# ubc-vision/quadraturefields

Hardware: AMD Instinct MI355X
Metric: rays/sec at 800x800 Lego (mesh-quadrature render: ray/mesh intersection + hash-grid/MLP field + compositing) (higher is better)
Workload: dtype f32; 1 GPU; Lego 800x800 (configs[1]), 1xMI355X per frame, fp32 hash-grid + tiny-MLP HIP kernels; rays_per_frame=640000, max_hits=25, triangles=983040, log2_hashmap_size=19, up_sample=1, bvh_fallback_frames=0, overflow_repaired_frames=8, reorigin_rule_redone_frames=0, camera_mismatch_frames=0, frames_in_flight=1

## Files before the change

### quadraturefields_amd/csrc/raster.hip

```cpp
#include <type_traits>

#include "exact_common.h"

#pragma clang fp contract(off)

namespace {

struct RasterCam {
    float r00, r01, r02, r10, r11, r12, r20, r21, r22;
    float cx, cy, cz;
    float fx, fy, px0, py0;
    int w, h;
};

constexpr float kRasterGuard = 0.25f;

struct SlabArgs {
    float t_lo, t_hi;
    int stop_at;
    uint64_t *keys;
    const float4 *ray_rec;
};

struct TriSetup {
    int x0, x1, y0, y1;
    bool use_edges;
    float ea[3], eb[3], ec[3];
};

__device__ __forceinline__ bool tri_setup(const float4 a, const float4 b, const float4 c, const RasterCam &cam, TriSetup &s)
{
    float minx = INFINITY, maxx = -INFINITY, miny = INFINITY, maxy = -INFINITY;
    int behind = 0;
    const float4 vs[3] = {a, b, c};
    float sxs[3], sys[3];
#pragma unroll
    for (int k = 0; k < 3; ++k) {
        const float dx = vs[k].x - cam.cx, dy = vs[k].y - cam.cy, dz = vs[k].z - cam.cz;
        const float xc = cam.r00 * dx + cam.r10 * dy + cam.r20 * dz;
        const float yc = cam.r01 * dx + cam.r11 * dy + cam.r21 * dz;
        const float zc = cam.r02 * dx + cam.r12 * dy + cam.r22 * dz;
        const float zv = -zc;
        if (!(zv > 1e-6f)) { ++behind; sxs[k] = sys[k] = 0.0f; continue; }
        const float sx = cam.fx * (xc / zv) + cam.px0;
        const float sy = -cam.fy * (yc / zv) + cam.py0;
        sxs[k] = sx; sys[k] = sy;
        minx = fminf(minx, sx); maxx = fmaxf(maxx, sx);
        miny = fminf(miny, sy); maxy = fmaxf(maxy, sy);
    }
    if (behind == 3) return false;
    s.use_edges = false;
    if (behind > 0) {
        s.x0 = 0; s.y0 = 0; s.x1 = cam.w - 1; s.y1 = cam.h - 1;
    } else {
        s.x0 = (int)fmaxf(floorf(minx - kRasterGuard), 0.0f);
        s.y0 = (int)fmaxf(floorf(miny - kRasterGuard), 0.0f);
        s.x1 = (int)fminf(ceilf(maxx + kRasterGuard), (float)(cam.w - 1));
        s.y1 = (int)fminf(ceilf(maxy + kRasterGuard), (float)(cam.h - 1));
        if (!(maxx + kRasterGuard >= 0.0f) || !(maxy + kRasterGuard >= 0.0f) ||
            !(minx - kRasterGuard <= (float)(cam.w - 1)) || !(miny - kRasterGuard <= (float)(cam.h - 1)))
            return false;
        const float area2 = (sxs[1] - sxs[0]) * (sys[2] - sys[0]) - (sys[1] - sys[0]) * (sxs[2] - sxs[0]);
        if (fabsf(area2) > 1e-2f) {
            s.use_edges = true;
            const float sgn = area2 > 0.0f ? 1.0f : -1.0f;
#pragma unroll
            for (int k = 0; k < 3; ++k) {
                const int k1 = (k + 1) % 3;
                const float ex = sxs[k1] - sxs[k], ey = sys[k1] - sys[k];
                s.ea[k] = -sgn * ey;
                s.eb[k] = sgn * ex;
                s.ec[k] = -(s.ea[k] * sxs[k] + s.eb[k] * sys[k]) + (kRasterGuard + 0.05f) * (fabsf(ex) + fabsf(ey)) + 1e-3f;
            }
        }
    }
    return true;
}

constexpr int kBinStage = 256;
constexpr int kBinIdBits = 26;
struct BinStage { int n; int tile[kBinStage]; uint2 rec[kBinStage]; };
struct TileBins {
    int32_t *cursor;
    uint2 *bins;
    int cap;
    BinStage *stage;
};

__device__ __forceinline__ void bin_records(const TileBins &tb, int tile, uint2 rec)
{
    const int lane = (int)__lane_id();
    for (;;) {
        const int t0 = __builtin_amdgcn_readfirstlane(tile);
        const unsigned long long m = __ballot(tile == t0);
        if (tile == t0) {
            const int rank = __popcll(m & ((1ull << lane) - 1ull));
            int base = 0;
            if (rank == 0) base = atomicAdd(&tb.cursor[t0], __popcll(m));
            base = __shfl(base, __ffsll((long long)m) - 1, 64);
            if (base + rank < tb.cap) tb.bins[(int64_t)t0 * tb.cap + base + rank] = rec;
            break;
        }
    }
}

template <int kRasterLanes, bool kWide, bool kSlab = false, bool kBins = false>
__device__ __forceinline__ void raster_triangle(const float4 *__restrict__ tris, int64_t tri_i, int sub, const RasterCam &cam,
                                                const float *__restrict__ rays_o, const float *__restrict__ rays_d,
                                                int max_hits, int32_t *__restrict__ hit_tri, float *__restrict__ hit_t,
                                                int32_t *__restrict__ hit_count, int32_t *__restrict__ overflow,
                                                const bool cam_origin, const SlabArgs slab = SlabArgs(),
                                                const TileBins bins = TileBins())
{
    const float4 a = tris[tri_i * 3 + 0], b = tris[tri_i * 3 + 1], c = tris[tri_i * 3 + 2];
    const int id = __float_as_int(a.w);
    TriSetup ts;
    if (!tri_setup(a, b, c, cam, ts)) return;
    const int x0 = ts.x0, x1 = ts.x1, y0 = ts.y0, y1 = ts.y1;
    const bool use_edges = ts.use_edges;
    const float *ea = ts.ea, *eb = ts.eb, *ec = ts.ec;
    const int bw = x1 - x0 + 1;
    const int total = bw * (y1 - y0 + 1);
    int px = x0 + sub % bw, py = y0 + sub / bw;
    for (int q = sub; q < total; q += kRasterLanes) {
        const int cx_ = px, cy_ = py;
        px += kRasterLanes;
        while (px > x1) { px -= bw; ++py; }
        if (use_edges) {
            const float fx_ = (float)cx_, fy_ = (float)cy_;
            if (ea[0] * fx_ + eb[0] * fy_ + ec[0] < 0.0f || ea[1] * fx_ + eb[1] * fy_ + ec[1] < 0.0f ||
                ea[2] * fx_ + eb[2] * fy_ + ec[2] < 0.0f)
                continue;
        }
        const int64_t ray = (int64_t)cy_ * cam.w + cx_;
        float dx, dy, dz;
        if (kSlab && slab.ray_rec) {
            const float4 rr = slab.ray_rec[ray];
            if (__float_as_int(rr.w) >= slab.stop_at) continue;
            dx = rr.x; dy = rr.y; dz = rr.z;
        } else {
            dx = rays_d[ray * 3]; dy = rays_d[ray * 3 + 1]; dz = rays_d[ray * 3 + 2];
        }
        float ox = cam.cx, oy = cam.cy, oz = cam.cz;
        if (!cam_origin) { ox = rays_o[ray * 3]; oy = rays_o[ray * 3 + 1]; oz = rays_o[ray * 3 + 2]; }
        asm volatile("" : "+v"(ox), "+v"(oy), "+v"(oz), "+v"(dx), "+v"(dy), "+v"(dz));
        float t;
        if (!mt_hit(a, b, c, ox, oy, oz, dx, dy, dz, &t)) continue;
        if (kSlab) {
            if (!(t >= slab.t_lo && t < slab.t_hi)) continue;
            const int slot = atomicAdd(&hit_count[ray], 1);
            if (slot < max_hits) slab.keys[(int64_t)slot * ((int64_t)cam.w * cam.h) + ray] = hit_key(t, id);
            else atomicAdd(overflow, 1);
            continue;
        }
        if (kBins) {
            const int tile = (cy_ >> 3) * ((cam.w + 7) >> 3) + (cx_ >> 3);
            const uint2 rec = make_uint2(__float_as_uint(t), ((uint32_t)id << 6) | (uint32_t)((cy_ & 7) * 8 + (cx_ & 7)));
            const int at = atomicAdd(&bins.stage->n, 1);
            if (at < kBinStage) { bins.stage->tile[at] = tile; bins.stage->rec[at] = rec; }
            else bin_records(bins, tile, rec);
            continue;
        }
        const int slot = atomicAdd(&hit_count[ray], 1);
        if (slot < max_hits) {
            const int64_t at = kWide ? (int64_t)slot * ((int64_t)cam.w * cam.h) + ray : ray * max_hits + slot;
            hit_t[at] = t;
            if (hit_tri) hit_tri[at] = id;
        } else {
            atomicAdd(overflow, 1);
        }
    }
}

template <int kRasterLanes, bool kWide>
__global__ __launch_bounds__(256) void raster_kernel(const float4 *__restrict__ tris, int64_t n_tri, RasterCam cam,
                                                     const float *__restrict__ rays_o, const float *__restrict__ rays_d,
                                                     int max_hits, int32_t *__restrict__ hit_tri, float *__restrict__ hit_t,
                                                     int32_t *__restrict__ hit_count, int32_t *__restrict__ overflow,
                                                     const int32_t *__restrict__ ray_flag)
{
    const int64_t gid = (int64_t)blockIdx.x * blockDim.x + threadIdx.x;
    const int64_t tri_i = gid / kRasterLanes;
    const int sub = (int)(gid % kRasterLanes);
    if (tri_i >= n_tri) return;
    if (ray_flag && *ray_flag) return;
    const bool cam_origin = ray_flag != nullptr;
    raster_triangle<kRasterLanes, kWide>(tris, tri_i, sub, cam, rays_o, rays_d, max_hits, hit_tri, hit_t, hit_count, overflow,
                                         cam_origin);
}

template <int kRasterLanes>
__global__ __launch_bounds__(256) void raster_bins_kernel(const float4 *__restrict__ tris, int64_t n_tri, RasterCam cam,
                                                          const float *__restrict__ rays_o, const float *__restrict__ rays_d,
                                                          int max_hits, int32_t *__restrict__ tile_cursor,
                                                          uint2 *__restrict__ bin_records_out,
                                                          const int32_t *__restrict__ ray_flag)
{
    __shared__ BinStage s_stage[4];
    const int64_t gid = (int64_t)blockIdx.x * blockDim.x + threadIdx.x;
    const int64_t tri_i = gid / kRasterLanes;
    const int sub = (int)(gid % kRasterLanes);
    if (ray_flag && *ray_flag) return;
    const bool cam_origin = ray_flag != nullptr;
    const int lane = (int)(threadIdx.x & 63);
    TileBins tb;
    tb.cursor = tile_cursor;
    tb.bins = bin_records_out;
    tb.cap = 64 * max_hits;
    tb.stage = &s_stage[threadIdx.x >> 6];
    if (lane == 0) tb.stage->n = 0;
    __builtin_amdgcn_fence(__ATOMIC_ACQ_REL, "workgroup");
    __builtin_amdgcn_wave_barrier();
    if (tri_i < n_tri)
        raster_triangle<kRasterLanes, false, false, true>(tris, tri_i, sub, cam, rays_o, rays_d, max_hits, nullptr, nullptr,
                                                          nullptr, nullptr, cam_origin, SlabArgs(), tb);
    __builtin_amdgcn_fence(__ATOMIC_ACQ_REL, "workgroup");
    __builtin_amdgcn_wave_barrier();
    const int n = tb.stage->n < kBinStage ? tb.stage->n : kBinStage;
    for (int i = lane; i < n; i += 64) bin_records(tb, tb.stage->tile[i], tb.stage->rec[i]);
}

__global__ __launch_bounds__(64) void tile_count_kernel(const int32_t *__restrict__ tile_cursor, const uint2 *__restrict__ bins,
                                                        int max_hits, int w, int h, int tiles_x,
                                                        int32_t *__restrict__ hit_count, int32_t *__restrict__ overflow,
                                                        uint64_t *__restrict__ tile_mask)
{
    __shared__ int s_cnt[64];
    const int tile = blockIdx.x, lane = threadIdx.x;
    const int cap = 64 * max_hits;
    const int cursor = tile_cursor[tile];
    const int n = cursor < cap ? cursor : cap;
    const int px = (tile % tiles_x) * 8 + (lane & 7), py = (tile / tiles_x) * 8 + (lane >> 3);
    const bool inside = px < w && py < h;
    int c = 0;
    if (n > 0) {
        s_cnt[lane] = 0;
        __syncthreads();
        const uint2 *run = bins + (int64_t)tile * cap;
        for (int i = lane; i < n; i += 64) atomicAdd(&s_cnt[run[i].y & 63u], 1);
        __syncthreads();
        c = s_cnt[lane];
    }
    int over = c > max_hits ? c - max_hits : 0;
    if (cursor > cap) {
        c = c > max_hits ? c : max_hits + 1;
        over = lane == 0 ? cursor - cap : 0;
    }
    if (inside) hit_count[(int64_t)py * w + px] = c;
    const unsigned long long mask = __ballot(inside && c > max_hits);
    if (mask) {
#pragma unroll
        for (int off = 32; off > 0; off >>= 1) over += __shfl_xor(over, off, 64);
        if (lane == 0) atomicAdd(overflow, over);
    }
    if (lane == 0) tile_mask[tile] = mask;
}

constexpr float kRayPixelTol = 0.02f;
constexpr float kRayUnitTol = 1e-4f;

__device__ __forceinline__ void camera_rays_check(const uint32_t *__restrict__ o_bits, const float *__restrict__ rays_d,
                                                  int64_t n_rays, const RasterCam &cam, int32_t *__restrict__ flag,
                                                  int64_t first, int64_t stride)
{
    const uint32_t c0 = __float_as_uint(cam.cx), c1 = __float_as_uint(cam.cy), c2 = __float_as_uint(cam.cz);
    bool bad = false;
    for (int64_t r = first; r < n_rays; r += stride) {
        const uint32_t o0 = o_bits[r * 3], o1 = o_bits[r * 3 + 1], o2 = o_bits[r * 3 + 2];
        const float dx = rays_d[r * 3], dy = rays_d[r * 3 + 1], dz = rays_d[r * 3 + 2];
        bad = bad || o0 != c0 || o1 != c1 || o2 != c2;
        const float xc = cam.r00 * dx + cam.r10 * dy + cam.r20 * dz;
        const float yc = cam.r01 * dx + cam.r11 * dy + cam.r21 * dz;
        const float zv = -(cam.r02 * dx + cam.r12 * dy + cam.r22 * dz);
        const float sx = cam.fx * (xc / zv) + cam.px0, sy = -cam.fy * (yc / zv) + cam.py0;
        const float px = (float)(int)(r % cam.w), py = (float)(int)(r / cam.w);
        bad = bad || !(zv > 0.0f) || !(fabsf(sx - px) <= kRayPixelTol) || !(fabsf(sy - py) <= kRayPixelTol) ||
              !(fabsf(dx * dx + dy * dy + dz * dz - 1.0f) <= kRayUnitTol);
    }
    if (bad) *flag = 1;
}

__global__ void camera_rays_check_kernel(const uint32_t *__restrict__ o_bits, const float *__restrict__ rays_d, int64_t n_rays,
                                         RasterCam cam, int32_t *__restrict__ flag)
{
    camera_rays_check(o_bits, rays_d, n_rays, cam, flag, (int64_t)blockIdx.x * blockDim.x + threadIdx.x,
                      (int64_t)gridDim.x * blockDim.x);
}

constexpr int kCullChunk = 64;

__global__ __launch_bounds__(256) void chunk_boxes_kernel(const float4 *__restrict__ tris, int64_t n_tri, int n_chunks,
                                                          float4 *__restrict__ boxes)
{
    const int chunk = (int)(((int64_t)blockIdx.x * blockDim.x + threadIdx.x) >> 6), lane = threadIdx.x & 63;
    if (chunk >= n_chunks) return;
    const int64_t t = (int64_t)chunk * kCullChunk + lane;
    float lo[3] = {INFINITY, INFINITY, INFINITY}, hi[3] = {-INFINITY, -INFINITY, -INFINITY};
    if (t < n_tri) {
#pragma unroll
        for (int k = 0; k < 3; ++k) {
            const float4 v = tris[t * 3 + k];
            lo[0] = fminf(lo[0], v.x); lo[1] = fminf(lo[1], v.y); lo[2] = fminf(lo[2], v.z);
            hi[0] = fmaxf(hi[0], v.x); hi[1] = fmaxf(hi[1], v.y); hi[2] = fmaxf(hi[2], v.z);
        }
    }
#pragma unroll
    for (int off = 32; off > 0; off >>= 1) {
#pragma unroll
        for (int k = 0; k < 3; ++k) {
            lo[k] = fminf(lo[k], __shfl_xor(lo[k], off, 64));
            hi[k] = fmaxf(hi[k], __shfl_xor(hi[k], off, 64));
        }
    }
    if (lane == 0) {
        boxes[chunk * 2 + 0] = make_float4(lo[0], lo[1], lo[2], 0.0f);
        boxes[chunk * 2 + 1] = make_float4(hi[0], hi[1], hi[2], 0.0f);
    }
}

__global__ void cull_chunks_kernel(const float4 *__restrict__ boxes, int n_chunks, RasterCam cam, int32_t *__restrict__ visible,
                                   int32_t *__restrict__ counters, int parity, const uint32_t *__restrict__ o_bits,
                                   const float *__restrict__ rays_d, int64_t n_rays, int32_t *__restrict__ ray_flag)
{
    const int chunk = blockIdx.x * blockDim.x + threadIdx.x;
    if (chunk == 0) counters[parity ^ 1] = 0;
    if (ray_flag) camera_rays_check(o_bits, rays_d, n_rays, cam, ray_flag, chunk, (int64_t)gridDim.x * blockDim.x);
    if (chunk >= n_chunks) return;
    const float4 lo = boxes[chunk * 2], hi = boxes[chunk * 2 + 1];
    if (!(lo.x <= hi.x)) return;
    float minx = INFINITY, maxx = -INFINITY, miny = INFINITY, maxy = -INFINITY;
    bool keep = false;
#pragma unroll
    for (int k = 0; k < 8; ++k) {
        const float dx = ((k & 1) ? hi.x : lo.x) - cam.cx, dy = ((k & 2) ? hi.y : lo.y) - cam.cy, dz = ((k & 4) ? hi.z : lo.z) - cam.cz;
        const float xc = cam.r00 * dx + cam.r10 * dy + cam.r20 * dz;
        const float yc = cam.r01 * dx + cam.r11 * dy + cam.r21 * dz;
        const float zc = cam.r02 * dx + cam.r12 * dy + cam.r22 * dz;
        const float zv = -zc;
        if (!(zv > 1e-4f)) { keep = true; continue; }
        const float sx = cam.fx * (xc / zv) + cam.px0, sy = -cam.fy * (yc / zv) + cam.py0;
        minx = fminf(minx, sx); maxx = fmaxf(maxx, sx);
        miny = fminf(miny, sy); maxy = fmaxf(maxy, sy);
    }
    const float g = kRasterGuard + 1.0f;
    if (!keep)
        keep = (maxx + g >= 0.0f) && (maxy + g >= 0.0f) && (minx - g <= (float)(cam.w - 1)) && (miny - g <= (float)(cam.h - 1));
    if (keep) visible[atomicAdd(&counters[parity], 1)] = chunk;
}

template <int kRasterLanes, bool kWide>
__global__ __launch_bounds__(256) void raster_culled_kernel(const float4 *__restrict__ tris, int64_t n_tri, RasterCam cam,
                                                            const float *__restrict__ rays_o, const float *__restrict__ rays_d,
                                                            int max_hits, int32_t *__restrict__ hit_tri, float *__restrict__ hit_t,
                                                            int32_t *__restrict__ hit_count, int32_t *__restrict__ overflow,
                                                            const int32_t *__restrict__ visible, const int32_t *__restrict__ n_visible,
                                                            const int32_t *__restrict__ ray_flag)
{
    if (ray_flag && *ray_flag) return;
    const bool cam_origin = ray_flag != nullptr;
    constexpr int kTrisPerBlock = 256 / kRasterLanes;
    constexpr int kBlocksPerChunk = kCullChunk / kTrisPerBlock;
    const int n_items = *n_visible * kBlocksPerChunk;
    const int sub = threadIdx.x % kRasterLanes;
    for (int item = blockIdx.x; item < n_items; item += gridDim.x) {
        const int chunk = visible[item / kBlocksPerChunk];
        const int64_t tri_i = (int64_t)chunk * kCullChunk + (item % kBlocksPerChunk) * kTrisPerBlock + threadIdx.x / kRasterLanes;
        if (tri_i < n_tri)
            raster_triangle<kRasterLanes, kWide>(tris, tri_i, sub, cam, rays_o, rays_d, max_hits, hit_tri, hit_t, hit_count, overflow,
                                                 cam_origin);
    }
}

// ... 372 lines not shown
        bvh->chunk_dirty = true;
        bvh->cull_parity = 0;
    }
    if (bvh->chunk_dirty) {
        hipLaunchKernelGGL(chunk_boxes_kernel, dim3((unsigned)qf_div_up(n_chunks * 64, 256)), dim3(256), 0, st,
                           reinterpret_cast<const float4 *>(bvh->d_tris), bvh->n_tri, (int)n_chunks,
                           reinterpret_cast<float4 *>(bvh->d_chunk_box));
        QF_LAUNCH_CHECK();
        bvh->chunk_dirty = false;
    }
    return QF_OK;
}

static int raster_zero(int64_t n_rays, int32_t *hit_count, int32_t *overflow, int32_t *origin_flag, hipStream_t st)
{
    int64_t words = n_rays;
    bool ovf_done = false, flag_done = origin_flag == nullptr;
    if (overflow == hit_count + words) { ++words; ovf_done = true; }
    if (ovf_done && origin_flag == hit_count + words) { ++words; flag_done = true; }
    QF_HIP_TRY(hipMemsetAsync(hit_count, 0, (size_t)words * sizeof(int32_t), st));
    if (!ovf_done) QF_HIP_TRY(hipMemsetAsync(overflow, 0, sizeof(int32_t), st));
    if (!flag_done) QF_HIP_TRY(hipMemsetAsync(origin_flag, 0, sizeof(int32_t), st));
    return QF_OK;
}

static int raster_lanes(int64_t n_rays, int64_t n_tri)
{
    const int64_t pixels_per_tri = n_rays / n_tri;
    return pixels_per_tri > 64 ? 16 : (pixels_per_tri > 8 ? 8 : 4);
}

template <typename F>
static void with_lanes(int lanes, F &&f)
{
    switch (lanes) {
    case 16: f(std::integral_constant<int, 16>()); break;
    case 8: f(std::integral_constant<int, 8>()); break;
    default: f(std::integral_constant<int, 4>()); break;
    }
}

static unsigned chunk_grid(int64_t n_chunks, int lanes)
{
    const int64_t items = n_chunks * (kCullChunk * lanes / 256);
    const int64_t cap = (int64_t)qf_cu_count_cached() * 8;
    return (unsigned)(items < cap ? items : cap);
}

static void camera_check_launch(const RasterCam &rc, const float *rays_o, const float *rays_d, int64_t n_rays,
                                int32_t *origin_flag, hipStream_t st)
{
    if (origin_flag)
        hipLaunchKernelGGL(camera_rays_check_kernel, dim3(qf_grid_1d(n_rays, 256)), dim3(256), 0, st,
                           reinterpret_cast<const uint32_t *>(rays_o), rays_d, n_rays, rc, origin_flag);
}

static int raster_launch(qf_bvh *bvh, const qf_camera *cam, const float *rays_o, const float *rays_d, int64_t n_rays,
                         int capacity, bool wide, int32_t *hit_tri, float *hit_t, int32_t *hit_count, int32_t *overflow,
                         int32_t *origin_flag, bool cull, hipStream_t st, bool skip_ids = false)
{
    if (skip_ids) hit_tri = nullptr;
    const int rc_zero = raster_zero(n_rays, hit_count, overflow, origin_flag, st);
    if (rc_zero != QF_OK) return rc_zero;
    if (bvh->n_tri == 0) return QF_OK;
    const RasterCam rc = make_raster_cam(cam);
    const float4 *tris4 = reinterpret_cast<const float4 *>(bvh->d_tris);
    const int lanes = raster_lanes(n_rays, bvh->n_tri);
    const int64_t blocks = qf_div_up(bvh->n_tri * lanes, 256);
    if (blocks > 0x7fffffff) return QF_ERR_UNSUPPORTED;
    if (cull) {
        const int64_t n_chunks = qf_div_up(bvh->n_tri, kCullChunk);
        const int rc_boxes = ensure_chunk_boxes(bvh, st);
        if (rc_boxes != QF_OK) return rc_boxes;
        float4 *boxes = reinterpret_cast<float4 *>(bvh->d_chunk_box);
        int32_t *counters = bvh->d_visible, *visible = bvh->d_visible + 2;
        const int parity = bvh->cull_parity;
        bvh->cull_parity ^= 1;
        bvh->cull_last = parity;
        hipLaunchKernelGGL(cull_chunks_kernel, dim3((unsigned)qf_div_up(n_chunks, 256)), dim3(256), 0, st, boxes,
                           (int)n_chunks, rc, visible, counters, parity, reinterpret_cast<const uint32_t *>(rays_o), rays_d,
                           n_rays, origin_flag);
        QF_LAUNCH_CHECK();
        with_lanes(lanes, [&](auto L) {
            auto *kernel = wide ? raster_culled_kernel<decltype(L)::value, true> : raster_culled_kernel<decltype(L)::value, false>;
            hipLaunchKernelGGL(kernel, dim3(chunk_grid(n_chunks, lanes)), dim3(256), 0, st, tris4, bvh->n_tri, rc, rays_o, rays_d,
                               capacity, hit_tri, hit_t, hit_count, overflow, visible, counters + parity, origin_flag);
        });
    } else {
        camera_check_launch(rc, rays_o, rays_d, n_rays, origin_flag, st);
        QF_LAUNCH_CHECK();
        with_lanes(lanes, [&](auto L) {
            auto *kernel = wide ? raster_kernel<decltype(L)::value, true> : raster_kernel<decltype(L)::value, false>;
            hipLaunchKernelGGL(kernel, dim3((unsigned)blocks), dim3(256), 0, st, tris4, bvh->n_tri, rc, rays_o, rays_d, capacity,
                               hit_tri, hit_t, hit_count, overflow, origin_flag);
        });
    }
    QF_LAUNCH_CHECK();
    return QF_OK;
}

static bool raster_args_ok(const qf_bvh *bvh, const qf_camera *cam, int64_t n_rays, int32_t max_hits)
{
    if (!bvh || !cam || n_rays < 0 || max_hits < 1 || max_hits > kMaxHits) return false;
    if (cam->width < 1 || cam->height < 1 || (int64_t)cam->width * cam->height != n_rays) return false;
    return cam->fx > 0.0f && cam->fy > 0.0f;
}

extern "C" int qf_raster_intersect(qf_bvh *bvh, const qf_camera *cam, const float *rays_o, const float *rays_d,
                                   int64_t n_rays, int32_t max_hits, int32_t *hit_tri, float *hit_t, int32_t *hit_count,
                                   int32_t *overflow, int32_t sort_lists, int32_t cull_chunks, int32_t *origin_flag,
                                   void *stream)
{
    if (!raster_args_ok(bvh, cam, n_rays, max_hits)) return QF_ERR_INVALID_ARGUMENT;
    if (!rays_o || !rays_d || !hit_tri || !hit_t || !hit_count || !overflow) return QF_ERR_INVALID_ARGUMENT;
    if (sort_lists < 0 || sort_lists > 2) return QF_ERR_INVALID_ARGUMENT;
    hipStream_t st = qf_stream(stream);
    const int rc = raster_launch(bvh, cam, rays_o, rays_d, n_rays, (int)max_hits, false, hit_tri, hit_t, hit_count, overflow,
                                 origin_flag, cull_chunks != 0, st, sort_lists == 2);
    if (rc != QF_OK) return rc;
    if (sort_lists == 1 && n_rays > 0) return filter_launch(n_rays, max_hits, bvh->min_sep, hit_tri, hit_t, hit_count, st);
    return QF_OK;
}

extern "C" int64_t qf_hit_bins_bytes(int32_t width, int32_t height, int32_t max_hits)
{
    if (width < 1 || height < 1 || max_hits < 1 || max_hits > kMaxHits) return -1;
    return (int64_t)((width + 7) / 8) * ((height + 7) / 8) * 64 * max_hits * (int64_t)sizeof(uint2);
}

extern "C" int qf_raster_intersect_tiles(qf_bvh *bvh, const qf_camera *cam, const float *rays_o, const float *rays_d,
                                         int64_t n_rays, int32_t max_hits, int32_t *tile_cursor, uint64_t *tile_mask,
                                         void *bins, int64_t bins_bytes, int32_t *hit_count, int32_t *overflow,
                                         int32_t *origin_flag, void *stream)
{
    if (!raster_args_ok(bvh, cam, n_rays, max_hits)) return QF_ERR_INVALID_ARGUMENT;
    if (!rays_o || !rays_d || !tile_cursor || !tile_mask || !bins || !hit_count || !overflow) return QF_ERR_INVALID_ARGUMENT;
    if (bins_bytes < qf_hit_bins_bytes(cam->width, cam->height, max_hits)) return QF_ERR_INVALID_ARGUMENT;
    if (reinterpret_cast<uintptr_t>(bins) % sizeof(uint2) || reinterpret_cast<uintptr_t>(tile_mask) % sizeof(uint64_t))
        return QF_ERR_INVALID_ARGUMENT;
    if (bvh->n_tri >= (1 << kBinIdBits)) return QF_ERR_UNSUPPORTED;
    hipStream_t st = qf_stream(stream);
    const int tiles_x = (cam->width + 7) / 8, n_tiles = tiles_x * ((cam->height + 7) / 8);
    QF_HIP_TRY(hipMemsetAsync(tile_cursor, 0, (size_t)n_tiles * sizeof(int32_t), st));
    if (origin_flag == overflow + 1) {
        QF_HIP_TRY(hipMemsetAsync(overflow, 0, 2 * sizeof(int32_t), st));
    } else {
        QF_HIP_TRY(hipMemsetAsync(overflow, 0, sizeof(int32_t), st));
        if (origin_flag) QF_HIP_TRY(hipMemsetAsync(origin_flag, 0, sizeof(int32_t), st));
    }
    const RasterCam rc = make_raster_cam(cam);
    uint2 *records = reinterpret_cast<uint2 *>(bins);
    if (bvh->n_tri > 0) {
        const int lanes = raster_lanes(n_rays, bvh->n_tri);
        const int64_t blocks = qf_div_up(bvh->n_tri * lanes, 256);
        if (blocks > 0x7fffffff) return QF_ERR_UNSUPPORTED;
        camera_check_launch(rc, rays_o, rays_d, n_rays, origin_flag, st);
        QF_LAUNCH_CHECK();
        with_lanes(lanes, [&](auto L) {
            hipLaunchKernelGGL(raster_bins_kernel<decltype(L)::value>, dim3((unsigned)blocks), dim3(256), 0, st,
                               reinterpret_cast<const float4 *>(bvh->d_tris), bvh->n_tri, rc, rays_o, rays_d, (int)max_hits,
                               tile_cursor, records, origin_flag);
        });
    }
    hipLaunchKernelGGL(tile_count_kernel, dim3((unsigned)n_tiles), dim3(64), 0, st, tile_cursor, records, (int)max_hits,
                       rc.w, rc.h, tiles_x, hit_count, overflow, tile_mask);
    QF_LAUNCH_CHECK();
    return QF_OK;
}

extern "C" int qf_raster_intersect_wide(qf_bvh *bvh, const qf_camera *cam, const float *rays_o, const float *rays_d,
                                        int64_t n_rays, int32_t max_hits, int32_t wide_hits, int32_t *wide_tri,
                                        float *wide_t, int32_t *hit_tri, float *hit_t, int32_t *hit_count,
                                        int32_t *overflow, int32_t cull_chunks, int32_t *origin_flag, void *stream)
{
    if (!raster_args_ok(bvh, cam, n_rays, max_hits)) return QF_ERR_INVALID_ARGUMENT;
    if (wide_hits < max_hits || wide_hits > 4096) return QF_ERR_INVALID_ARGUMENT;
    if (!rays_o || !rays_d || !wide_tri || !wide_t || !hit_tri || !hit_t || !hit_count || !overflow)
        return QF_ERR_INVALID_ARGUMENT;
    hipStream_t st = qf_stream(stream);
    const int rc = raster_launch(bvh, cam, rays_o, rays_d, n_rays, (int)wide_hits, true, wide_tri, wide_t, hit_count, overflow,
                                 origin_flag, cull_chunks != 0, st);
    if (rc != QF_OK) return rc;
    if (n_rays == 0) return QF_OK;
    const size_t lds = (size_t)select_capacity(max_hits, wide_hits, bvh->min_sep) * kSelectBlock * 2 * sizeof(float);
    hipLaunchKernelGGL(select_nearest_kernel<false>, dim3((unsigned)qf_div_up(n_rays, kSelectBlock)), dim3(kSelectBlock), lds, st,
                       n_rays, (int)wide_hits, (int)max_hits, bvh->min_sep, wide_tri, wide_t, (const uint64_t *)nullptr, hit_tri,
                       hit_t, hit_count);
    QF_LAUNCH_CHECK();
    return QF_OK;
}

extern "C" int qf_raster_intersect_slabs(qf_bvh *bvh, const qf_camera *cam, const float *rays_o, const float *rays_d,
                                         int64_t n_rays, int32_t max_hits, int32_t wide_hits, int32_t n_slabs,
                                         uint64_t *wide_keys, int32_t *hit_tri, float *hit_t, int32_t *hit_count,
                                         int32_t *overflow, int32_t *origin_flag, void *stream)
{
    if (!raster_args_ok(bvh, cam, n_rays, max_hits)) return QF_ERR_INVALID_ARGUMENT;
    if (n_slabs < 2 || n_slabs > kMaxSlabs) return QF_ERR_INVALID_ARGUMENT;
    const int sel_cap = select_capacity(max_hits, wide_hits, bvh->min_sep);
    if (wide_hits <= sel_cap + 1 || wide_hits > 4096) return QF_ERR_INVALID_ARGUMENT;
    if (!rays_o || !rays_d || !wide_keys || !hit_tri || !hit_t || !hit_count || !overflow) return QF_ERR_INVALID_ARGUMENT;
    hipStream_t st = qf_stream(stream);
    const int rc_zero = raster_zero(n_rays, hit_count, overflow, origin_flag, st);
    if (rc_zero != QF_OK) return rc_zero;
    if (n_rays == 0 || bvh->n_tri == 0) return QF_OK;
    const int rc_boxes = ensure_chunk_boxes(bvh, st);
    if (rc_boxes != QF_OK) return rc_boxes;
    const int64_t n_chunks = qf_div_up(bvh->n_tri, kCullChunk);
    if (!bvh->d_slab_range) {
        QF_HIP_TRY(hipMalloc((void **)&bvh->d_slab_range, (size_t)n_chunks * sizeof(float2)));
        QF_HIP_TRY(hipMalloc((void **)&bvh->d_slab_lists, (size_t)n_chunks * kMaxSlabs * sizeof(int32_t)));
        QF_HIP_TRY(hipMalloc((void **)&bvh->d_slab_ctl, sizeof(SlabCtl)));
    }
    const RasterCam rc = make_raster_cam(cam);
    const float4 *tris4 = reinterpret_cast<const float4 *>(bvh->d_tris);
    const float4 *boxes = reinterpret_cast<const float4 *>(bvh->d_chunk_box);
    int32_t *visible = bvh->d_visible + 2;
    bvh->cull_last = -1;
    float2 *range = reinterpret_cast<float2 *>(bvh->d_slab_range);
    SlabCtl *ctl = reinterpret_cast<SlabCtl *>(bvh->d_slab_ctl);
    camera_check_launch(rc, rays_o, rays_d, n_rays, origin_flag, st);
    hipLaunchKernelGGL(slab_init_kernel, dim3(1), dim3(1), 0, st, ctl);
    hipLaunchKernelGGL(slab_cull_kernel, dim3((unsigned)qf_div_up(n_chunks, 256)), dim3(256), 0, st, boxes, (int)n_chunks, rc,
                       visible, range, ctl);
    hipLaunchKernelGGL(slab_assign_kernel, dim3((unsigned)qf_div_up(n_chunks, 256)), dim3(256), 0, st, visible, range, ctl,
                       (int)n_slabs, (int)n_chunks, bvh->d_slab_lists);
    QF_LAUNCH_CHECK();
    const int lanes = raster_lanes(n_rays, bvh->n_tri);
    const unsigned grid = chunk_grid(n_chunks, lanes);
    const int stop_at = sel_cap + 1;
    if (bvh->slab_snapshot_rays < n_rays) {
        const int64_t grown = bvh->slab_snapshot_rays * 2 > n_rays ? bvh->slab_snapshot_rays * 2 : n_rays;
        if (bvh->d_slab_snapshot) (void)hipFree(bvh->d_slab_snapshot);
        bvh->d_slab_snapshot = nullptr;
        bvh->slab_snapshot_rays = 0;
        QF_HIP_TRY(hipMalloc((void **)&bvh->d_slab_snapshot, (size_t)grown * sizeof(float4)));
        bvh->slab_snapshot_rays = grown;
    }
    float4 *snapshot = reinterpret_cast<float4 *>(bvh->d_slab_snapshot);
    for (int j = 0; j < n_slabs; ++j) {
        if (j > 0) {
            hipLaunchKernelGGL(slab_ray_records_kernel, dim3(qf_grid_1d(n_rays, 256)), dim3(256), 0, st, rays_d, hit_count,
                               n_rays, snapshot);
            QF_LAUNCH_CHECK();
        }
        const int32_t *list = bvh->d_slab_lists + (int64_t)j * n_chunks;
        with_lanes(lanes, [&](auto L) {
            hipLaunchKernelGGL(raster_slab_kernel<decltype(L)::value>, dim3(grid), dim3(256), 0, st, tris4, bvh->n_tri, rc, rays_o,
                               rays_d, (int)wide_hits, wide_keys, hit_count, overflow, list, ctl, j, (int)n_slabs, stop_at,
                               j == 0 ? (const float4 *)nullptr : snapshot, origin_flag);
        });
    }
    QF_LAUNCH_CHECK();
    const size_t lds = (size_t)sel_cap * kSelectBlock * 2 * sizeof(float);
    hipLaunchKernelGGL(select_nearest_kernel<true>, dim3((unsigned)qf_div_up(n_rays, kSelectBlock)), dim3(kSelectBlock), lds, st,
                       n_rays, (int)wide_hits, (int)max_hits, bvh->min_sep, (const int32_t *)nullptr, (const float *)nullptr,
                       wide_keys, hit_tri, hit_t, hit_count);
    QF_LAUNCH_CHECK();
    return QF_OK;
}

extern "C" int64_t qf_bvh_copy_visible_chunks(const qf_bvh *bvh, int32_t *chunks_host, int64_t capacity, void *stream)
{
    if (!bvh || capacity < 0 || (capacity > 0 && !chunks_host)) return QF_ERR_INVALID_ARGUMENT;
    if (!bvh->d_visible || bvh->cull_last < 0) return QF_ERR_INVALID_ARGUMENT;
    QF_HIP_TRY(hipStreamSynchronize(qf_stream(stream)));
    int32_t n = 0;
    QF_HIP_TRY(hipMemcpy(&n, bvh->d_visible + bvh->cull_last, sizeof(int32_t), hipMemcpyDeviceToHost));
    const int64_t n_chunks = qf_div_up(bvh->n_tri, kCullChunk);
    if (n < 0 || n > n_chunks) return QF_ERR_HIP;
    const int64_t take = n < capacity ? n : capacity;
    if (take > 0) QF_HIP_TRY(hipMemcpy(chunks_host, bvh->d_visible + 2, (size_t)take * sizeof(int32_t), hipMemcpyDeviceToHost));
    return n;
}
```

### quadraturefields_amd/csrc/sample_pack.hip

```cpp
#include "exact_common.h"

#pragma clang fp contract(off)

namespace {

template <int kN, bool kTri>
__device__ __forceinline__ void sort_to_row(float (&t)[kN], int32_t (&id)[kN], int cnt, float *row_t, int32_t *row_i)
{
    if (kTri) {
        uint64_t key[kN];
#pragma unroll
        for (int k = 0; k < kN; ++k) key[k] = k < cnt ? hit_key(t[k], id[k]) : ~0ull;
#pragma unroll
        for (int k = 2; k <= kN; k <<= 1) {
#pragma unroll
            for (int i = 0; i < kN; ++i) {
                const int l = i ^ (k - 1);
                if (l > i) { const uint64_t a = key[i], b = key[l]; key[i] = a < b ? a : b; key[l] = a < b ? b : a; }
            }
#pragma unroll
            for (int j = k >> 2; j > 0; j >>= 1) {
#pragma unroll
                for (int i = 0; i < kN; ++i) {
                    const int l = i ^ j;
// ... 197 lines not shown
        const double d64[3] = {(double)dx, (double)dy, (double)dz};
        double p[3];
        const double dep = sample_depth64(s_t[rl * Kp + k], o64, d64, p);
        const float nrm = sqrtf((dx * dx + dy * dy) + dz * dz) + 1e-7f;
        const int64_t o = block_base + j;
        if (xyz) {
            xyz[o * 3 + 0] = (float)p[0];
            xyz[o * 3 + 1] = (float)p[1];
            xyz[o * 3 + 2] = (float)p[2];
            dirs[o * 3 + 0] = dx / nrm;
            dirs[o * 3 + 1] = dy / nrm;
            dirs[o * 3 + 2] = dz / nrm;
            origins[o * 3 + 0] = ox;
            origins[o * 3 + 1] = oy;
            origins[o * 3 + 2] = oz;
        }
        index_ray[o] = ray;
        depth[o] = (float)dep;
        index_tri[o] = (int64_t)s_tri[rl * Kp + k];
        if (inverse) {
            const int64_t c = inverse[o];
            xyz_c[c * 3 + 0] = (float)p[0];
            xyz_c[c * 3 + 1] = (float)p[1];
            xyz_c[c * 3 + 2] = (float)p[2];
            dirs_c[c * 3 + 0] = dx / nrm;
            dirs_c[c * 3 + 1] = dy / nrm;
            dirs_c[c * 3 + 2] = dz / nrm;
            if (depth_c) depth_c[c] = (float)dep;
        }
    }
}

template <bool kTri, bool kBins>
__global__ __launch_bounds__(64) void pack_tiles_kernel(
    const float *__restrict__ rays_o, const float *__restrict__ rays_d, int w, int h, int tiles_x, int n_tiles, int max_hits,
    const int32_t *__restrict__ hit_tri, const float *__restrict__ hit_t, const int32_t *__restrict__ hit_count,
    const int64_t *__restrict__ tile_base, const int64_t *__restrict__ total, float *__restrict__ xyz_c,
    float *__restrict__ dirs_c, float *__restrict__ depth_c, int32_t *__restrict__ tri_c, const uint64_t *__restrict__ keep_mask,
    const int32_t *__restrict__ raw_count, float min_sep, int32_t *__restrict__ final_count, int32_t *__restrict__ dropped,
    const int32_t *__restrict__ tile_cursor, const uint64_t *__restrict__ tile_mask, const uint2 *__restrict__ bins,
    const int32_t *__restrict__ ray_flag)
{
    extern __shared__ __attribute__((aligned(16))) unsigned char smem[];
    const int K = max_hits, Kp = max_hits | 1;
    float *s_t = reinterpret_cast<float *>(smem);
    int32_t *s_tri = reinterpret_cast<int32_t *>(s_t + 64 * Kp);
    const int tile = blockIdx.x, lane = threadIdx.x;
    const int px0 = (tile % tiles_x) * 8, py0 = (tile / tiles_x) * 8;
    const int cols = (w - px0) < 8 ? (w - px0) : 8, rows = (h - py0) < 8 ? (h - py0) : 8;
    const int px = px0 + (lane & 7), py = py0 + (lane >> 3);
    const bool inside = px < w && py < h;
    const int64_t ray = inside ? (int64_t)py * w + px : 0;
    int cnt = 0;
    if (inside) {
        cnt = keep_mask ? raw_count[ray] : hit_count[ray];
        if (cnt > K) cnt = K;
    }
    int deepest = cnt;
#pragma unroll
    for (int off = 32; off > 0; off >>= 1) {
        const int other = __shfl_xor(deepest, off, 64);
        deepest = other > deepest ? other : deepest;
    }
    if (deepest == 0) {
        if (final_count && inside) final_count[ray] = 0;
        return;
    }
    float *row_t = s_t + lane * Kp;
    int32_t *row_i = s_tri + lane * Kp;
    const float ox = rays_o[ray * 3], oy = rays_o[ray * 3 + 1], oz = rays_o[ray * 3 + 2];
    const float dx = rays_d[ray * 3], dy = rays_d[ray * 3 + 1], dz = rays_d[ray * 3 + 2];
    int64_t base = tile_base[tile];
    if (kBins) {
        __shared__ int s_fill[64];
        const unsigned long long by_row = (ray_flag && *ray_flag) ? ~0ull : tile_mask[tile];
        const int cap = 64 * K;
        const int cursor = tile_cursor[tile];
        const int n = by_row == ~0ull ? 0 : (cursor < cap ? cursor : cap);
        const uint2 *run = bins + (int64_t)tile * cap;
        s_fill[lane] = 0;
        __syncthreads();
        for (int i = lane; i < n; i += 64) {
            const uint2 rec = run[i];
            const int p = (int)(rec.y & 63u);
            const int at = atomicAdd(&s_fill[p], 1);
            if (!((by_row >> p) & 1ull) && at < K) {
                s_t[p * Kp + at] = __uint_as_float(rec.x);
                if (kTri) s_tri[p * Kp + at] = (int32_t)(rec.y >> 6);
            }
        }
        __syncthreads();
        const bool own_row = (by_row >> lane) & 1ull;
        if (deepest <= 16) {
            if (own_row) load_sort_row<16, kTri>(hit_t + ray * K, hit_tri + ray * K, K, cnt, deepest, row_t, row_i);
            else sort_row_in_place<16, kTri>(cnt, deepest, row_t, row_i);
        } else {
            if (own_row) load_sort_row<32, kTri>(hit_t + ray * K, hit_tri + ray * K, K, cnt, deepest, row_t, row_i);
            else sort_row_in_place<32, kTri>(cnt, deepest, row_t, row_i);
        }
    } else if (K <= 32) {
        if (deepest <= 16) load_sort_row<16, kTri>(hit_t + ray * K, hit_tri + ray * K, K, cnt, deepest, row_t, row_i);
        else load_sort_row<32, kTri>(hit_t + ray * K, hit_tri + ray * K, K, cnt, deepest, row_t, row_i);
    } else {
        for (int yy = 0; yy < rows; ++yy) {
            const int64_t row_ray0 = (int64_t)(py0 + yy) * w + px0;
            for (int i = lane; i < cols * deepest; i += 64) {
                const int r = i / deepest, k = i - r * deepest;
                s_t[(yy * 8 + r) * Kp + k] = hit_t[(row_ray0 + r) * K + k];
                if (kTri) s_tri[(yy * 8 + r) * Kp + k] = hit_tri[(row_ray0 + r) * K + k];
            }
        }
        __syncthreads();
    }
    double o64[3] = {0.0, 0.0, 0.0}, d64[3] = {0.0, 0.0, 0.0};
    float dn[3] = {0.0f, 0.0f, 0.0f};
    int n_dropped = 0;
    if (inside) {
        if (K > 32) {
            for (int i = 1; i < cnt; ++i) {
                const float t = row_t[i];
                const int id = kTri ? row_i[i] : 0;
                int j = i - 1;
                while (j >= 0 && (kTri ? hit_less(t, id, row_t[j], row_i[j]) : t < row_t[j])) {
                    row_t[j + 1] = row_t[j];
                    if (kTri) row_i[j + 1] = row_i[j];
                    --j;
                }
                row_t[j + 1] = t;
                if (kTri) row_i[j + 1] = id;
            }
        }
        if (keep_mask) {
            const uint64_t mask = keep_mask[ray];
            int kept = 0;
            for (int i = 0; i < cnt; ++i)
                if ((mask >> i) & 1ull) { row_t[kept] = row_t[i]; if (kTri) row_i[kept] = row_i[i]; ++kept; }
            cnt = kept;
        } else if (min_sep > 0.0f && cnt > 1) {
            float last_t = row_t[0];
            int kept = 1;
            for (int i = 1; i < cnt; ++i) {
                const float t = row_t[i];
                if (t > last_t + min_sep) { row_t[kept] = t; if (kTri) row_i[kept] = row_i[i]; ++kept; last_t = t; }
            }
            n_dropped = cnt - kept;
            cnt = kept;
        }
        if (cnt > 0) {
            o64[0] = (double)ox; o64[1] = (double)oy; o64[2] = (double)oz;
            d64[0] = (double)dx; d64[1] = (double)dy; d64[2] = (double)dz;
            const float nrm = sqrtf((dx * dx + dy * dy) + dz * dz) + 1e-7f;
            dn[0] = dx / nrm; dn[1] = dy / nrm; dn[2] = dz / nrm;
        }
        if (cnt > 1) {
            double p[3];
            double prev = sample_depth64(row_t[0], o64, d64, p);
            bool sorted = true;
            for (int k = 1; k < cnt; ++k) {
                const double dk = sample_depth64(row_t[k], o64, d64, p);
                sorted = sorted && !(prev > dk);
                prev = dk;
            }
            if (!sorted) {
                for (int i = 1; i < cnt; ++i) {
                    const float t = row_t[i];
                    const int id = kTri ? row_i[i] : 0;
                    const double di = sample_depth64(t, o64, d64, p);
                    int j = i - 1;
                    while (j >= 0 && sample_depth64(row_t[j], o64, d64, p) > di) {
                        row_t[j + 1] = row_t[j];
                        if (kTri) row_i[j + 1] = row_i[j];
                        --j;
                    }
                    row_t[j + 1] = t;
                    if (kTri) row_i[j + 1] = id;
                }
            }
        }
    }
    if (final_count && inside) final_count[ray] = cnt;
    const unsigned long long below = (1ull << lane) - 1ull;
    float first_xyz[3] = {0.0f, 0.0f, 0.0f};
    for (int k = 0;; ++k) {
        const unsigned long long mask = __ballot(cnt > k);
        if (mask == 0ull) break;
        if (cnt > k) {
            const int64_t c = base + __popcll(mask & below);
            double p[3];
            const double dep = sample_depth64(row_t[k], o64, d64, p);
            xyz_c[c * 3 + 0] = (float)p[0];
            xyz_c[c * 3 + 1] = (float)p[1];
            xyz_c[c * 3 + 2] = (float)p[2];
            dirs_c[c * 3 + 0] = dn[0];
            dirs_c[c * 3 + 1] = dn[1];
            dirs_c[c * 3 + 2] = dn[2];
            depth_c[c] = (float)dep;
            if (kTri) tri_c[c] = (int32_t)row_i[k];
            if (k == 0) { first_xyz[0] = (float)p[0]; first_xyz[1] = (float)p[1]; first_xyz[2] = (float)p[2]; }
        }
        base += __popcll(mask);
    }
    const unsigned long long any_drop = __ballot(n_dropped > 0);
    if (any_drop) {
        const int64_t end = tile + 1 < n_tiles ? tile_base[tile + 1] : *total;
        const int src = __ffsll((long long)__ballot(cnt > 0)) - 1;
        const float gx = __shfl(first_xyz[0], src, 64), gy = __shfl(first_xyz[1], src, 64), gz = __shfl(first_xyz[2], src, 64);
        const float hx = __shfl(dn[0], src, 64), hy = __shfl(dn[1], src, 64), hz = __shfl(dn[2], src, 64);
        const int gtri = kTri ? __shfl((int)row_i[0], src, 64) : 0;
        for (int64_t c = base + lane; c < end; c += 64) {
            xyz_c[c * 3 + 0] = gx; xyz_c[c * 3 + 1] = gy; xyz_c[c * 3 + 2] = gz;
            dirs_c[c * 3 + 0] = hx; dirs_c[c * 3 + 1] = hy; dirs_c[c * 3 + 2] = hz;
            depth_c[c] = 0.0f;
            if (kTri) tri_c[c] = (int32_t)gtri;
        }
        int sum = n_dropped;
#pragma unroll
        for (int off = 32; off > 0; off >>= 1) sum += __shfl_xor(sum, off, 64);
        if (lane == 0 && dropped) atomicAdd(dropped, sum);
    }
}

__global__ void publish_dropped_kernel(int32_t *dropped, int64_t *host_out)
{
    host_out[2] = (int64_t)*dropped;
    *dropped = 0;
}

__global__ void resort_kernel(const int64_t *index_ray, const float *depth, int64_t n, int64_t *perm)
{
    for (int64_t i = (int64_t)blockIdx.x * blockDim.x + threadIdx.x; i < n; i += (int64_t)gridDim.x * blockDim.x) {
        const int64_t ray = index_ray[i];
        if (i != 0 && index_ray[i - 1] == ray) continue;
        perm[i] = i;
        for (int64_t k = i + 1; k < n && index_ray[k] == ray; ++k) {
            const float dk = depth[k];
            int64_t j = k - 1;
            while (j >= i && depth[perm[j]] > dk) { perm[j + 1] = perm[j]; --j; }
            perm[j + 1] = k;
        }
    }
}

constexpr int RS_THREADS = 256;
constexpr int RS_CHUNK = 1024;
constexpr int RS_HALO = 64;
constexpr int RS_STAGE = RS_CHUNK + RS_HALO;

__global__ __launch_bounds__(RS_THREADS) void resort_samples_kernel(
    const int64_t *index_ray, const float *depth, int64_t n, const float *points, const float *origins,
    const float *vectors, const int64_t *index_tri, int64_t *perm, float *out_points, float *out_depth,
    float *out_origins, float *out_vectors, int64_t *out_index_tri, uint8_t *boundary, const int32_t *inverse,
    float *out_points_c, float *out_vectors_c)
{
    __shared__ float s_depth[RS_STAGE];
    __shared__ int64_t s_ray[RS_STAGE + 1];
    __shared__ int s_src[RS_STAGE];
    __shared__ uint8_t s_mine[RS_STAGE];
    __shared__ int s_heads[RS_CHUNK];
    __shared__ int s_nheads;
    const int64_t n_chunks = (n + RS_CHUNK - 1) / RS_CHUNK;
    for (int64_t chunk = blockIdx.x; chunk < n_chunks; chunk += gridDim.x) {
        const int64_t b0 = chunk * RS_CHUNK;
        const int staged = (int)((n - b0 < RS_STAGE) ? (n - b0) : RS_STAGE);
        const int own = (int)((n - b0 < RS_CHUNK) ? (n - b0) : RS_CHUNK);
        if (threadIdx.x == 0) {
            s_ray[0] = b0 > 0 ? index_ray[b0 - 1] : 0;
            s_nheads = 0;
        }
        for (int k = threadIdx.x; k < staged; k += RS_THREADS) {
            s_depth[k] = depth[b0 + k];
            s_ray[k + 1] = index_ray[b0 + k];
            s_mine[k] = 0;
        }
        __syncthreads();
        for (int k = threadIdx.x; k < own; k += RS_THREADS) {
            const bool head = (b0 + k == 0) || s_ray[k] != s_ray[k + 1];
            if (boundary) boundary[b0 + k] = head ? 1 : 0;
            if (head) s_heads[atomicAdd(&s_nheads, 1)] = k;
        }
        __syncthreads();
        const int n_heads = s_nheads;
        for (int h = threadIdx.x; h < n_heads; h += RS_THREADS) {
            const int k = s_heads[h];
            const int64_t ray = s_ray[k + 1];
            int end = k + 1;
            while (end < staged && s_ray[end + 1] == ray) ++end;
            const bool spills = end == staged && b0 + staged < n && index_ray[b0 + staged] == ray;
            if (!spills) {
                s_src[k] = k;
                s_mine[k] = 1;
                for (int q = k + 1; q < end; ++q) {
                    const float dq = s_depth[q];
                    int j = q - 1;
                    while (j >= k && s_depth[s_src[j]] > dq) { s_src[j + 1] = s_src[j]; --j; }
                    s_src[j + 1] = q;
                    s_mine[q] = 1;
                }
            } else {
                const int64_t i = b0 + k;
                int64_t e = i + 1;
                while (e < n && index_ray[e] == ray) ++e;
                for (int64_t q = i; q < e; ++q) {
                    const float dq = depth[q];
                    int64_t rank = 0;
                    for (int64_t r = i; r < e; ++r) {
                        const float dr = depth[r];
                        rank += (dr < dq) || (dr == dq && r < q);
                    }
                    const int64_t dst = i + rank;
                    if (perm) perm[dst] = q;
                    out_depth[dst] = dq;
                    if (out_index_tri) out_index_tri[dst] = index_tri[q];
                    const int64_t pos_c = inverse ? (int64_t)inverse[dst] : 0;
                    for (int c = 0; c < 3; ++c) {
                        out_points[dst * 3 + c] = points[q * 3 + c];
                        if (out_origins) out_origins[dst * 3 + c] = origins[q * 3 + c];
                        out_vectors[dst * 3 + c] = vectors[q * 3 + c];
                        if (inverse) {
                            out_points_c[pos_c * 3 + c] = points[q * 3 + c];
                            out_vectors_c[pos_c * 3 + c] = vectors[q * 3 + c];
                        }
                    }
                }
            }
        }
        __syncthreads();
        for (int k = threadIdx.x; k < staged; k += RS_THREADS) {
            if (!s_mine[k]) continue;
            const int64_t src = b0 + s_src[k], dst = b0 + k;
            if (perm) perm[dst] = src;
            out_depth[dst] = s_depth[s_src[k]];
            if (out_index_tri) out_index_tri[dst] = index_tri[src];
        }
        for (int e = threadIdx.x; e < 3 * staged; e += RS_THREADS) {
            const int k = e / 3, c = e - 3 * k;
            if (!s_mine[k]) continue;
            const int64_t src = (b0 + s_src[k]) * 3 + c, dst = b0 * 3 + e;
            const float pv = points[src], vv = vectors[src];
            out_points[dst] = pv;
            if (out_origins) out_origins[dst] = origins[src];
            out_vectors[dst] = vv;
            if (inverse) {
                const int64_t pc = (int64_t)inverse[b0 + k] * 3 + c;
                out_points_c[pc] = pv;
                out_vectors_c[pc] = vv;
            }
        }
        __syncthreads();
    }
}

}

// ... 112 lines not shown
```

Baseline: 408.4 million rays/s.

## Share per-triangle setup across block runs and fold sortedness check into sample emission

The bin rasterizer now assigns a run of 64 triangles per block. One wave computes the triangle setups (bounding box, edge equations) once into shared memory, and all waves then loop over rounds of pixel work, flushing the per-wave staging buffer after each round. Before, each triangle's setup was recomputed redundantly by every sub-lane. Separately, sample packing no longer runs a double-precision depth pass just to check sort order; it checks while emitting samples and redoes the emission only for waves with unsorted rows. That adds a second write pass in the rare unsorted case and more barriers and shared-memory use in the raster kernel.

Result: no change. 410.4 million rays/s, median of 3 (+0.5%).

```diff
diff --git a/quadraturefields_amd/csrc/raster.hip b/quadraturefields_amd/csrc/raster.hip
--- a/quadraturefields_amd/csrc/raster.hip
+++ b/quadraturefields_amd/csrc/raster.hip
@@ -1,6 +1,7 @@
 #include <type_traits>
 
 #include "exact_common.h"
+#include "raster_runs.h"
 
 #pragma clang fp contract(off)
 
@@ -105,17 +106,14 @@
 }
 
 template <int kRasterLanes, bool kWide, bool kSlab = false, bool kBins = false>
-__device__ __forceinline__ void raster_triangle(const float4 *__restrict__ tris, int64_t tri_i, int sub, const RasterCam &cam,
-                                                const float *__restrict__ rays_o, const float *__restrict__ rays_d,
-                                                int max_hits, int32_t *__restrict__ hit_tri, float *__restrict__ hit_t,
-                                                int32_t *__restrict__ hit_count, int32_t *__restrict__ overflow,
-                                                const bool cam_origin, const SlabArgs slab = SlabArgs(),
-                                                const TileBins bins = TileBins())
-{
-    const float4 a = tris[tri_i * 3 + 0], b = tris[tri_i * 3 + 1], c = tris[tri_i * 3 + 2];
+__device__ __forceinline__ void raster_pixels(const float4 a, const float4 b, const float4 c, const TriSetup &ts, int sub,
+                                              const RasterCam &cam, const float *__restrict__ rays_o,
+                                              const float *__restrict__ rays_d, int max_hits, int32_t *__restrict__ hit_tri,
+                                              float *__restrict__ hit_t, int32_t *__restrict__ hit_count,
+                                              int32_t *__restrict__ overflow, const bool cam_origin, const SlabArgs slab,
+                                              const TileBins bins)
+{
     const int id = __float_as_int(a.w);
-    TriSetup ts;
-    if (!tri_setup(a, b, c, cam, ts)) return;
     const int x0 = ts.x0, x1 = ts.x1, y0 = ts.y0, y1 = ts.y1;
     const bool use_edges = ts.use_edges;
     const float *ea = ts.ea, *eb = ts.eb, *ec = ts.ec;
@@ -172,6 +170,20 @@
     }
 }
 
+template <int kRasterLanes, bool kWide, bool kSlab = false>
+__device__ __forceinline__ void raster_triangle(const float4 *__restrict__ tris, int64_t tri_i, int sub, const RasterCam &cam,
+                                                const float *__restrict__ rays_o, const float *__restrict__ rays_d,
+                                                int max_hits, int32_t *__restrict__ hit_tri, float *__restrict__ hit_t,
+                                                int32_t *__restrict__ hit_count, int32_t *__restrict__ overflow,
+                                                const bool cam_origin, const SlabArgs slab = SlabArgs())
+{
+    const float4 a = tris[tri_i * 3 + 0], b = tris[tri_i * 3 + 1], c = tris[tri_i * 3 + 2];
+    TriSetup ts;
+    if (!tri_setup(a, b, c, cam, ts)) return;
+    raster_pixels<kRasterLanes, kWide, kSlab, false>(a, b, c, ts, sub, cam, rays_o, rays_d, max_hits, hit_tri, hit_t, hit_count,
+                                                     overflow, cam_origin, slab, TileBins());
+}
+
 template <int kRasterLanes, bool kWide>
 __global__ __launch_bounds__(256) void raster_kernel(const float4 *__restrict__ tris, int64_t n_tri, RasterCam cam,
                                                      const float *__restrict__ rays_o, const float *__restrict__ rays_d,
@@ -189,35 +201,78 @@
                                          cam_origin);
 }
 
+constexpr int kRunWaves = 4;
+struct RunSetup {
+    int flags[kRasterRun];
+    int x0[kRasterRun], x1[kRasterRun], y0[kRasterRun], y1[kRasterRun];
+    float ea[3][kRasterRun], eb[3][kRasterRun], ec[3][kRasterRun];
+};
+
 template <int kRasterLanes>
-__global__ __launch_bounds__(256) void raster_bins_kernel(const float4 *__restrict__ tris, int64_t n_tri, RasterCam cam,
-                                                          const float *__restrict__ rays_o, const float *__restrict__ rays_d,
-                                                          int max_hits, int32_t *__restrict__ tile_cursor,
-                                                          uint2 *__restrict__ bin_records_out,
-                                                          const int32_t *__restrict__ ray_flag)
-{
-    __shared__ BinStage s_stage[4];
-    const int64_t gid = (int64_t)blockIdx.x * blockDim.x + threadIdx.x;
-    const int64_t tri_i = gid / kRasterLanes;
-    const int sub = (int)(gid % kRasterLanes);
+__global__ __launch_bounds__(64 * kRunWaves, 8) void raster_bins_kernel(const float4 *__restrict__ tris, int64_t n_tri,
+                                                                        RasterCam cam, const float *__restrict__ rays_o,
+                                                                        const float *__restrict__ rays_d, int max_hits,
+                                                                        int32_t *__restrict__ tile_cursor,
+                                                                        uint2 *__restrict__ bin_records_out,
+                                                                        const int32_t *__restrict__ ray_flag)
+{
+    static_assert(kRasterRun == 64 && kRasterRun % kRasterLanes == 0, "one triangle per lane, whole triangles per round");
+    __shared__ BinStage s_stage[kRunWaves];
+    __shared__ RunSetup su;
     if (ray_flag && *ray_flag) return;
     const bool cam_origin = ray_flag != nullptr;
-    const int lane = (int)(threadIdx.x & 63);
+    const int lane = (int)(threadIdx.x & 63), wave = (int)(threadIdx.x >> 6);
+    const int64_t first = qf_raster_run_first(blockIdx.x);
+    const int in_run = qf_raster_run_count(n_tri, first);
     TileBins tb;
     tb.cursor = tile_cursor;
     tb.bins = bin_records_out;
     tb.cap = 64 * max_hits;
-    tb.stage = &s_stage[threadIdx.x >> 6];
+    tb.stage = &s_stage[wave];
     if (lane == 0) tb.stage->n = 0;
-    __builtin_amdgcn_fence(__ATOMIC_ACQ_REL, "workgroup");
-    __builtin_amdgcn_wave_barrier();
-    if (tri_i < n_tri)
-        raster_triangle<kRasterLanes, false, false, true>(tris, tri_i, sub, cam, rays_o, rays_d, max_hits, nullptr, nullptr,
-                                                          nullptr, nullptr, cam_origin, SlabArgs(), tb);
-    __builtin_amdgcn_fence(__ATOMIC_ACQ_REL, "workgroup");
-    __builtin_amdgcn_wave_barrier();
-    const int n = tb.stage->n < kBinStage ? tb.stage->n : kBinStage;
-    for (int i = lane; i < n; i += 64) bin_records(tb, tb.stage->tile[i], tb.stage->rec[i]);
+    if (wave == 0) {
+        int flags = 0;
+        if (lane < in_run) {
+            const int64_t tri_i = first + lane;
+            TriSetup ts;
+            if (tri_setup(tris[tri_i * 3 + 0], tris[tri_i * 3 + 1], tris[tri_i * 3 + 2], cam, ts)) {
+                flags = ts.use_edges ? 3 : 1;
+                su.x0[lane] = ts.x0; su.x1[lane] = ts.x1; su.y0[lane] = ts.y0; su.y1[lane] = ts.y1;
+                if (ts.use_edges) {
+#pragma unroll
+                    for (int k = 0; k < 3; ++k) { su.ea[k][lane] = ts.ea[k]; su.eb[k][lane] = ts.eb[k]; su.ec[k][lane] = ts.ec[k]; }
+                }
+            }
+        }
+        su.flags[lane] = flags;
+    }
+    __syncthreads();
+    for (int round = wave; round < kRasterLanes; round += kRunWaves) {
+        const QfRunSlot slot = qf_raster_run_slot(round, lane, kRasterLanes);
+        const int flags = su.flags[slot.tri];
+        if (__ballot(flags != 0) == 0ull) continue;
+        if (flags != 0) {
+            TriSetup ts;
+            ts.x0 = su.x0[slot.tri]; ts.x1 = su.x1[slot.tri]; ts.y0 = su.y0[slot.tri]; ts.y1 = su.y1[slot.tri];
+            ts.use_edges = (flags & 2) != 0;
+            if (ts.use_edges) {
+#pragma unroll
+                for (int k = 0; k < 3; ++k) { ts.ea[k] = su.ea[k][slot.tri]; ts.eb[k] = su.eb[k][slot.tri]; ts.ec[k] = su.ec[k][slot.tri]; }
+            }
+            const int64_t tri_i = first + slot.tri;
+            raster_pixels<kRasterLanes, false, false, true>(tris[tri_i * 3 + 0], tris[tri_i * 3 + 1], tris[tri_i * 3 + 2], ts,
+                                                            slot.sub, cam, rays_o, rays_d, max_hits, nullptr, nullptr, nullptr,
+                                                            nullptr, cam_origin, SlabArgs(), tb);
+        }
+        __builtin_amdgcn_fence(__ATOMIC_ACQ_REL, "workgroup");
+        __builtin_amdgcn_wave_barrier();
+        const int n = tb.stage->n < kBinStage ? tb.stage->n : kBinStage;
+        for (int i = lane; i < n; i += 64) bin_records(tb, tb.stage->tile[i], tb.stage->rec[i]);
+        __builtin_amdgcn_wave_barrier();
+        if (lane == 0) tb.stage->n = 0;
+        __builtin_amdgcn_fence(__ATOMIC_ACQ_REL, "workgroup");
+        __builtin_amdgcn_wave_barrier();
+    }
 }
 
 __global__ __launch_bounds__(64) void tile_count_kernel(const int32_t *__restrict__ tile_cursor, const uint2 *__restrict__ bins,
@@ -896,12 +951,12 @@
     uint2 *records = reinterpret_cast<uint2 *>(bins);
     if (bvh->n_tri > 0) {
         const int lanes = raster_lanes(n_rays, bvh->n_tri);
-        const int64_t blocks = qf_div_up(bvh->n_tri * lanes, 256);
+        const int64_t blocks = qf_raster_run_blocks(bvh->n_tri);
         if (blocks > 0x7fffffff) return QF_ERR_UNSUPPORTED;
         camera_check_launch(rc, rays_o, rays_d, n_rays, origin_flag, st);
         QF_LAUNCH_CHECK();
         with_lanes(lanes, [&](auto L) {
-            hipLaunchKernelGGL(raster_bins_kernel<decltype(L)::value>, dim3((unsigned)blocks), dim3(256), 0, st,
+            hipLaunchKernelGGL(raster_bins_kernel<decltype(L)::value>, dim3((unsigned)blocks), dim3(64 * kRunWaves), 0, st,
                                reinterpret_cast<const float4 *>(bvh->d_tris), bvh->n_tri, rc, rays_o, rays_d, (int)max_hits,
                                tile_cursor, records, origin_flag);
         });
diff --git a/quadraturefields_amd/csrc/raster_runs.h b/quadraturefields_amd/csrc/raster_runs.h
--- /dev/null
+++ b/quadraturefields_amd/csrc/raster_runs.h
@@ -0,0 +1,32 @@
+#pragma once
+#include <stdint.h>
+
+#ifdef __HIPCC__
+#define QF_RUN_FN __host__ __device__ __forceinline__
+#else
+#define QF_RUN_FN inline
+#endif
+
+constexpr int kRasterRun = 64;
+
+QF_RUN_FN int64_t qf_raster_run_blocks(int64_t n_tri) { return n_tri > 0 ? (n_tri + kRasterRun - 1) / kRasterRun : 0; }
+
+QF_RUN_FN int64_t qf_raster_run_first(int64_t block) { return block * kRasterRun; }
+
+QF_RUN_FN int qf_raster_run_count(int64_t n_tri, int64_t first)
+{
+    const int64_t left = n_tri - first;
+    return left < 0 ? 0 : (left < kRasterRun ? (int)left : kRasterRun);
+}
+
+struct QfRunSlot {
+    int tri, sub;
+};
+
+QF_RUN_FN QfRunSlot qf_raster_run_slot(int round, int lane, int lanes)
+{
+    QfRunSlot s;
+    s.tri = (kRasterRun / lanes) * round + lane / lanes;
+    s.sub = lane % lanes;
+    return s;
+}
diff --git a/quadraturefields_amd/csrc/sample_pack.hip b/quadraturefields_amd/csrc/sample_pack.hip
--- a/quadraturefields_amd/csrc/sample_pack.hip
+++ b/quadraturefields_amd/csrc/sample_pack.hip
@@ -373,53 +373,54 @@
             const float nrm = sqrtf((dx * dx + dy * dy) + dz * dz) + 1e-7f;
             dn[0] = dx / nrm; dn[1] = dy / nrm; dn[2] = dz / nrm;
         }
-        if (cnt > 1) {
-            double p[3];
-            double prev = sample_depth64(row_t[0], o64, d64, p);
-            bool sorted = true;
-            for (int k = 1; k < cnt; ++k) {
-                const double dk = sample_depth64(row_t[k], o64, d64, p);
-                sorted = sorted && !(prev > dk);
-                prev = dk;
-            }
-            if (!sorted) {
-                for (int i = 1; i < cnt; ++i) {
-                    const float t = row_t[i];
-                    const int id = kTri ? row_i[i] : 0;
-                    const double di = sample_depth64(t, o64, d64, p);
-                    int j = i - 1;
-                    while (j >= 0 && sample_depth64(row_t[j], o64, d64, p) > di) {
-                        row_t[j + 1] = row_t[j];
-                        if (kTri) row_i[j + 1] = row_i[j];
-                        --j;
-                    }
-                    row_t[j + 1] = t;
-                    if (kTri) row_i[j + 1] = id;
-                }
-            }
-        }
     }
     if (final_count && inside) final_count[ray] = cnt;
     const unsigned long long below = (1ull << lane) - 1ull;
     float first_xyz[3] = {0.0f, 0.0f, 0.0f};
-    for (int k = 0;; ++k) {
-        const unsigned long long mask = __ballot(cnt > k);
-        if (mask == 0ull) break;
-        if (cnt > k) {
-            const int64_t c = base + __popcll(mask & below);
+    bool unsorted = false;
+    for (int pass = 0;; ++pass) {
+        int64_t at = base;
+        double prev = 0.0;
+        for (int k = 0;; ++k) {
+            const unsigned long long mask = __ballot(cnt > k);
+            if (mask == 0ull) break;
+            if (cnt > k && (pass == 0 || unsorted)) {
+                const int64_t c = at + __popcll(mask & below);
+                double p[3];
+                const double dep = sample_depth64(row_t[k], o64, d64, p);
+                if (pass == 0) { unsorted = unsorted || prev > dep; prev = dep; }
+                xyz_c[c * 3 + 0] = (float)p[0];
+                xyz_c[c * 3 + 1] = (float)p[1];
+                xyz_c[c * 3 + 2] = (float)p[2];
+                dirs_c[c * 3 + 0] = dn[0];
+                dirs_c[c * 3 + 1] = dn[1];
+                dirs_c[c * 3 + 2] = dn[2];
+                depth_c[c] = (float)dep;
+                if (kTri) tri_c[c] = (int32_t)row_i[k];
+                if (k == 0) { first_xyz[0] = (float)p[0]; first_xyz[1] = (float)p[1]; first_xyz[2] = (float)p[2]; }
+            }
+            at += __popcll(mask);
+        }
+        if (pass == 1 || __ballot(unsorted) == 0ull) {
+            base = at;
+            break;
+        }
+        if (unsorted) {
             double p[3];
-            const double dep = sample_depth64(row_t[k], o64, d64, p);
-            xyz_c[c * 3 + 0] = (float)p[0];
-            xyz_c[c * 3 + 1] = (float)p[1];
-            xyz_c[c * 3 + 2] = (float)p[2];
-            dirs_c[c * 3 + 0] = dn[0];
-            dirs_c[c * 3 + 1] = dn[1];
-            dirs_c[c * 3 + 2] = dn[2];
-            depth_c[c] = (float)dep;
-            if (kTri) tri_c[c] = (int32_t)row_i[k];
-            if (k == 0) { first_xyz[0] = (float)p[0]; first_xyz[1] = (float)p[1]; first_xyz[2] = (float)p[2]; }
-        }
-        base += __popcll(mask);
+            for (int i = 1; i < cnt; ++i) {
+                const float t = row_t[i];
+                const int id = kTri ? row_i[i] : 0;
+                const double di = sample_depth64(t, o64, d64, p);
+                int j = i - 1;
+                while (j >= 0 && sample_depth64(row_t[j], o64, d64, p) > di) {
+                    row_t[j + 1] = row_t[j];
+                    if (kTri) row_i[j + 1] = row_i[j];
+                    --j;
+                }
+                row_t[j + 1] = t;
+                if (kTri) row_i[j + 1] = id;
+            }
+        }
     }
     const unsigned long long any_drop = __ballot(n_dropped > 0);
     if (any_drop) {
```
